# feldroop/genedex

Measured on AMD Instinct MI355X. Metric: queries/sec (count+locate), hg38-scale text, 100M len-50 reads, higher is better.
Workload: dtype u32

## Files before the change

### genedex_amd/csrc/search.hip

```cpp
#include <atomic>
#include <cstdlib>
#include <string>
#include <type_traits>

#include "common.hpp"
#include "kernels.hpp"

namespace gdx {

namespace {

constexpr int kBlock = 256;

struct QueryWindow {
    const uint64_t *words;
    uint64_t cur;
    uint64_t next;
    uint64_t cur_word;
    uint64_t first_word;

    __device__ __forceinline__ void init(const uint8_t *qbuf, uint64_t begin, uint64_t pos)
    {
        words = reinterpret_cast<const uint64_t *>(qbuf);
        first_word = begin >> 3;
// ... 2708 lines not shown
            s_pr[wave][at] = rem;
            s_pc[wave][at] = make_uint2(static_cast<uint32_t>(qcode), static_cast<uint32_t>(qcode >> 32));
        }
        n_parked += static_cast<uint32_t>(__popcll(mask));
    };
    auto goes_on = [&](const u32x4 &en, uint32_t tagd) __attribute__((always_inline)) {
        return (en.x & kSeedFound) == 0u && (en.x & kSeedOverflow) != 0u && (tagd >> kSeedDispShift) < kSeedMaxDisp;
    };
    auto parked_pass = [&]() __attribute__((always_inline)) {
        const uint32_t take = n_parked < 64u ? n_parked : 64u;
        const uint32_t first = n_parked - take;
        __builtin_amdgcn_wave_barrier();
        const bool mine = lane < take;
        uint32_t q = 0, bucket = 0, tagd = kNoTag, rem = 0;
        uint64_t qcode = 0;
        if (mine) {
            q = s_pq[wave][first + lane];
            bucket = s_pb[wave][first + lane];
            tagd = s_pt[wave][first + lane];
            rem = s_pr[wave][first + lane];
            const uint2 c = s_pc[wave][first + lane];
            qcode = (static_cast<uint64_t>(c.y) << 32) | c.x;
        }
        __builtin_amdgcn_wave_barrier();
        n_parked = first;
        s_bt[wave][lane] = make_uint2(bucket, tagd);
        const u32x4 en = gather();
        const bool again = mine && goes_on(en, tagd);
        const uint32_t kind = (mine && !again) ? finish(q, rem, qcode, en) : 0u;
        if (kind == 1u && tile_sums != nullptr) {
            const uint32_t t = q / kSumTile - tile0;
            if (t < 2u) atomicAdd(&s_tile_hits[t], 1u);
            else atomicAdd(&tile_sums[q / kSumTile], 1ull);
        }
        list_late(kind, q);
        park(again, q, bucket, tagd, rem, qcode);
    };

    const uint64_t n_ranges = (nq + range - 1) / range;
    for (uint64_t rg = blockIdx.x; rg < n_ranges; rg += gridDim.x) {
        const uint64_t base = rg * range;
        const uint32_t cnt = nq - base < range ? static_cast<uint32_t>(nq - base) : range;
        const uint32_t n_chunks = (cnt + 63u) >> 6;
        tile0 = static_cast<uint32_t>(base / kSumTile);
        uint64_t r_end = 0;
        uint32_t r_len = 0;
        bool r_on = false, r_load = false;
        uint32_t raw[kRaw];
#pragma unroll
        for (int i = 0; i < kRaw; i++) raw[i] = 0u;
        auto fetch = [&](uint32_t ch) __attribute__((always_inline)) {
            const uint32_t slot = ch * 64u + lane;
            r_on = ch < n_chunks && slot < cnt;
            r_load = false;
            if (!r_on) return;
            const uint64_t q = base + slot;
            uint64_t beg;
            if (kUniform) {
                beg = q * ulen;
                r_end = beg + ulen;
            } else {
                beg = qbeg[q];
                r_end = qend[q];
            }
            const uint64_t len = r_end - beg;
            r_len = len < (1ull << 21) ? static_cast<uint32_t>(len) : (1u << 21);
            r_load = r_len >= k && r_len < (1u << 21) && r_end >= kWin;
            if (!r_load) return;
            if (kXlate == 2) {
                const uint64_t bit = 2ull * (r_end - kWin);
                const uint32_t *p = qw + (bit >> 5);
                const u32x4_a4 v = *reinterpret_cast<const u32x4_a4 *>(p);
                raw[0] = v.x, raw[1] = v.y, raw[2] = v.z, raw[3] = v.w;
                raw[4] = p[4];
            } else {
                const uint32_t *p1 = qw + ((r_end - kWin) >> 2);
                const u32x4_a4 *p = reinterpret_cast<const u32x4_a4 *>(p1);
#pragma unroll
                for (int i = 0; i < 3; i++) {
                    const u32x4_a4 v = p[i];
                    raw[4 * i] = v.x, raw[4 * i + 1] = v.y, raw[4 * i + 2] = v.z, raw[4 * i + 3] = v.w;
                }
                raw[12] = p1[12];
                raw[13] = p1[13];
                raw[14] = ((r_end - kWin) & 3u) != 0u ? p1[14] : 0u;
            }
        };
        fetch(wave);
        for (uint32_t ch = wave; ch < n_chunks; ch += kWaves) {
            const uint32_t q = static_cast<uint32_t>(base + ch * 64u + lane);
            const bool on = r_on;
            bool left = on && !r_load;
            const uint32_t rem = r_len - k;
            uint32_t f0 = 0, f1 = 0, f2 = 0, f3 = 0;
            if (kXlate == 2) {
                const uint32_t sh = static_cast<uint32_t>(2ull * (r_end - kWin)) & 31u;
                f0 = __builtin_amdgcn_alignbit(raw[1], raw[0], sh);
                f1 = __builtin_amdgcn_alignbit(raw[2], raw[1], sh);
                f2 = __builtin_amdgcn_alignbit(raw[3], raw[2], sh);
                f3 = __builtin_amdgcn_alignbit(raw[4], raw[3], sh);
            } else {
                const uint32_t o = static_cast<uint32_t>(r_end - kWin) & 3u;
                const uint32_t lo = kWin - (r_len < span ? r_len : span);
                uint32_t bad = 0, c[14];
#pragma unroll
                for (uint32_t i = 0; i < 14; i++) {
                    const uint32_t bytes = __builtin_amdgcn_alignbyte(raw[i + 1], raw[i], o);
                    uint32_t b = 0;
                    c[i] = fast_pack4(sv, bytes, b);
                    const uint32_t m = 4u * i + 4u <= lo ? 0u : (4u * i >= lo ? 0xffffffffu : 0xffffffffu << (8u * (lo - 4u * i)));
                    bad |= b & m;
                }
                f0 = c[0] | (c[1] << 8) | (c[2] << 16) | (c[3] << 24);
                f1 = c[4] | (c[5] << 8) | (c[6] << 16) | (c[7] << 24);
                f2 = c[8] | (c[9] << 8) | (c[10] << 16) | (c[11] << 24);
                f3 = c[12] | (c[13] << 8);
                if (bad != 0u) left = on;
            }
            const uint64_t wq = (static_cast<uint64_t>(f1) << 32) | f0, wk = (static_cast<uint64_t>(f3) << 32) | f2;
            const uint64_t qcode0 = drop2 == 0u ? wq : (wq >> drop2) | (wk << (64u - drop2));
            const uint64_t key = (wk >> drop2) & ((1ull << (2u * k)) - 1ull);
            uint32_t tag = 0;
            const uint32_t bucket = seed_home(key, sv.tag_bits, sv.buckets, tag);
            const bool look = on && !left;
            s_bt[wave][lane] = look ? make_uint2(bucket, tag) : make_uint2(0u, kNoTag);
            s_qc[wave][lane] = make_uint2(static_cast<uint32_t>(qcode0), static_cast<uint32_t>(qcode0 >> 32));
            fetch(ch + kWaves);
            const u32x4 en = gather();
            uint32_t li = lane;
            asm volatile("" : "+v"(li));
            const uint2 qc2 = s_qc[wave][li];
            const uint64_t qcode = (static_cast<uint64_t>(qc2.y) << 32) | qc2.x;
            if (left) {
                if (state) state[q] = make_uint4(0u, 0u, 0u, 0u);
                if (out_compact) out_compact[q] = kCompactSee;
            }
            const bool again = look && goes_on(en, tag);
            const uint32_t kind = left ? kListLeft : ((look && !again) ? finish(q, rem, qcode, en) : 0u);
            list_slot(kind, ch * 64u + lane);
            if (tile_sums != nullptr) {
                const unsigned long long hm = __ballot(kind == 1u);
                if (lane == 0u && hm != 0ull)
                    atomicAdd(&s_tile_hits[static_cast<uint32_t>((base + ch * 64u) / kSumTile) - tile0], static_cast<uint32_t>(__popcll(hm)));
            }
            park(again, q, bucket, tag, rem, qcode);
            while (n_parked >= 64u) parked_pass();
        }
        if (rg + gridDim.x >= n_ranges)
            while (n_parked != 0u) parked_pass();
        flush_lists(base);
    }
}

template <int kXlate, bool kExact>
__global__ __launch_bounds__(kBlock) void seed_text_kernel4(
    SeedView sv, const uint8_t *__restrict__ qbuf, const uint64_t *__restrict__ qbeg, const uint32_t *__restrict__ list,
    const uint32_t *__restrict__ n_list, const uint2 *__restrict__ long_state, uint32_t long_stride,
    uint32_t *__restrict__ out_count, uint8_t *__restrict__ out_status, uint4 *__restrict__ out_rec,
    uint32_t *__restrict__ out_start, uint32_t *__restrict__ out_end, uint32_t *__restrict__ out_compact,
    uint4 *__restrict__ state, uint32_t *__restrict__ leftover, uint32_t *__restrict__ n_leftover, uint32_t ulen)
{
    constexpr uint32_t kGroup = 4, kGroups = kBlock / kGroup;
    __shared__ uint8_t s_dense[256];
    if (kXlate == 0) {
        for (int i = threadIdx.x; i < 256; i += kBlock) s_dense[i] = sv.io_to_dense[i];
        __syncthreads();
    }
    const uint32_t sub = threadIdx.x & (kGroup - 1u);
    const bool writer = sub == 0u;
    const uint64_t n = *n_list;
    for (uint64_t i = static_cast<uint64_t>(blockIdx.x) * kGroups + threadIdx.x / kGroup; i < n;
         i += static_cast<uint64_t>(gridDim.x) * kGroups) {
        const uint32_t q = list[i];
        uint32_t pos, rem;
        if (kExact) {
            pos = out_start[q];
            rem = out_end[q];
        } else {
            const uint2 st = long_state[static_cast<uint64_t>(q) * long_stride];
            pos = st.x;
            rem = st.y;
        }
        const uint64_t begin = query_begin(qbeg, ulen, q);
        const uint32_t rest = rem - 32u;
        uint32_t bad_q = 0, bad_t = 0;
        for (uint32_t done = 0; done < rest; done += 128u) {
            const uint32_t skip = done + 32u * sub;
            if (skip < rest) {
                const uint32_t e = rest - skip, n_c = e < 32u ? e : 32u, qs = e - n_c;
                const uint64_t at = begin + qs;
                const uint64_t s0 = static_cast<uint64_t>(pos) - rem + qs + 32u * kTextPadUnits;
                const uint32_t tb = static_cast<uint32_t>(s0 & 31u);
                const u32x4 *tu = sv.text_units + (s0 >> 5);
                uint64_t qc = 0;
                uint32_t inv = 0;
                u32x4 u0, u1;
                if (kXlate == 2) {
                    const uint16_t *up = reinterpret_cast<const uint16_t *>(qbuf) + (at >> 3);
                    const uint32_t sh = static_cast<uint32_t>(at & 7u) * 2u;
                    const uint32_t n_need = (static_cast<uint32_t>(at & 7u) + n_c + 7u) >> 3;
                    uint64_t lo64 = up[0];
                    uint32_t hi16 = 0;
                    if (n_need > 1u) lo64 |= static_cast<uint64_t>(up[1]) << 16;
                    if (n_need > 2u) lo64 |= static_cast<uint64_t>(up[2]) << 32;
                    if (n_need > 3u) lo64 |= static_cast<uint64_t>(up[3]) << 48;
                    if (n_need > 4u) hi16 = up[4];
                    u0 = tu[0];
                    u1 = tb != 0u ? tu[1] : u32x4{0u, 0u, 0u, 0u};
                    qc = sh != 0u ? (lo64 >> sh) | (static_cast<uint64_t>(hi16) << (64u - sh)) : lo64;
                } else {
                const uint64_t *wp = reinterpret_cast<const uint64_t *>(qbuf) + (at >> 3);
                const uint32_t sh = static_cast<uint32_t>(at & 7u) * 8u;
                const uint32_t n_need = (static_cast<uint32_t>(at & 7u) + n_c + 7u) >> 3;
                uint64_t w0 = wp[0], w1 = 0, w2 = 0, w3 = 0, w4 = 0;
                if (n_need > 1u) w1 = wp[1];
                if (n_need > 2u) w2 = wp[2];
                if (n_need > 3u) w3 = wp[3];
                if (n_need > 4u) w4 = wp[4];
                u0 = tu[0];
                u1 = tb != 0u ? tu[1] : u32x4{0u, 0u, 0u, 0u};
                if (sh != 0u) {
                    w0 = (w0 >> sh) | (w1 << (64u - sh));
                    w1 = (w1 >> sh) | (w2 << (64u - sh));
                    w2 = (w2 >> sh) | (w3 << (64u - sh));
                    w3 = (w3 >> sh) | (w4 << (64u - sh));
                }
                uint32_t b[8] = {0u, 0u, 0u, 0u, 0u, 0u, 0u, 0u};
                const uint32_t wd[8] = {static_cast<uint32_t>(w0), static_cast<uint32_t>(w0 >> 32), static_cast<uint32_t>(w1),
                                        static_cast<uint32_t>(w1 >> 32), static_cast<uint32_t>(w2), static_cast<uint32_t>(w2 >> 32),
                                        static_cast<uint32_t>(w3), static_cast<uint32_t>(w3 >> 32)};
#pragma unroll
                for (uint32_t g = 0; g < 8; g++) {
                    const uint32_t code = kXlate == 1 ? fast_pack4(sv, wd[g], b[g]) : fast_pack4_lds(s_dense, wd[g], b[g]);
                    qc |= static_cast<uint64_t>(code) << (8u * g);
                }
                const uint32_t full = n_c >> 2, part = n_c & 3u;
#pragma unroll
                for (uint32_t g = 0; g < 8; g++) {
                    const uint32_t bg = kXlate == 1 ? b[g] : (b[g] != 0u ? 0xffffffffu : 0u);
                    if (g < full) inv |= bg;
                    else if (g == full && part != 0u) inv |= bg & ((1u << (8u * part)) - 1u);
                }
                }
                const uint64_t c0 = static_cast<uint64_t>(u0.x) | (static_cast<uint64_t>(u0.y) << 32);
                const uint64_t c1 = static_cast<uint64_t>(u1.x) | (static_cast<uint64_t>(u1.y) << 32);
                const uint64_t tc = tb ? (c0 >> (2u * tb)) | (c1 << (64u - 2u * tb)) : c0;
                const uint32_t tm = tb ? (u0.z >> tb) | (u1.z << (32u - tb)) : u0.z;
                const uint64_t m64 = n_c == 32u ? ~0ull : (1ull << (2u * n_c)) - 1ull;
                const uint32_t m32 = n_c == 32u ? ~0u : (1u << n_c) - 1u;
                if (inv != 0u) bad_q = 1u;
                if (((qc ^ tc) & m64) != 0ull || (tm & m32) != 0u) bad_t = 1u;
            }
        }
        const bool left = group_max<kGroup>(bad_q) != 0u;
        const bool hit = group_max<kGroup>(bad_t) == 0u;
        if (kExact) {
            if (left || !hit) {
                if (writer) leftover[atomicAdd(n_leftover, 1u)] = q;
            } else {
                const uint32_t row = sv.isa[pos - rem];
                if (writer) {
                    out_start[q] = row;
                    out_end[q] = row + 1u;
                    if (out_count) out_count[q] = 1u;
                    if (out_status) out_status[q] = 0;
                }
            }
        } else if (writer) {
            if (left) {
                leftover[atomicAdd(n_leftover, 1u)] = q;
                if (state) state[q] = make_uint4(0u, 0u, 0u, 0u);
                if (out_compact) out_compact[q] = kCompactSee;
            } else {
                if (out_compact) out_compact[q] = hit ? pos - rem : kCompactNone;
                else if (out_rec) out_rec[q] = hit ? make_uint4(0u, 1u, pos - rem, kRecResolved) : make_uint4(0u, 0u, 0xffffffffu, 0u);
                if (out_count) out_count[q] = hit ? 1u : 0u;
                if (out_status) out_status[q] = 0;
            }
        }
    }
}

template <int kJump, int kMode>
__global__ __launch_bounds__(kBlock) __attribute__((amdgpu_waves_per_eu(7, 7))) void search_pair_packed_kernel4(GDX_SEARCH_ARGS)
{
    search_pair_body<0, 4, false, kJump, kMode, true>(GDX_SEARCH_FWD);
}
template <int kPolicy, int kJump, int kMode>
__global__ __launch_bounds__(kBlock) void search_pair_stats_kernel8(GDX_SEARCH_ARGS)
{
    search_pair_body<kPolicy, 8, true, kJump, kMode>(GDX_SEARCH_FWD);
}
template <int kPolicy, int kJump, int kMode>
__global__ __launch_bounds__(kBlock) void search_pair_stats_kernel4(GDX_SEARCH_ARGS)
{
    search_pair_body<kPolicy, 4, true, kJump, kMode>(GDX_SEARCH_FWD);
}

template <class Table, int kGroup, bool kPair>
__global__ __launch_bounds__(kBlock) void extend_front_kernel(IndexView ix, uint32_t *__restrict__ start,
                                                              uint32_t *__restrict__ end,
                                                              const uint8_t *__restrict__ io_symbols, uint64_t m,
                                                              uint8_t *__restrict__ out_status)
{
    const uint64_t stride = static_cast<uint64_t>(gridDim.x) * (kBlock / kGroup);
    const bool writer = (threadIdx.x % kGroup) == 0;
    for (uint64_t i = static_cast<uint64_t>(blockIdx.x) * (kBlock / kGroup) + threadIdx.x / kGroup; i < m; i += stride) {
        uint32_t lo = start[i], hi = end[i];
        const uint32_t c = ix.io_to_dense[io_symbols[i]];
        uint32_t status = GDX_Q_OK;
        if (c == 0) {
            status = GDX_Q_INVALID_SYMBOL;
        } else if (lo != hi) {
            if (kPair && c <= 4u) {
                PairTable::lf1<1, 8>(ix, c, lo, hi, lo, hi);
            } else {
                uint32_t rlo, rhi;
                Table::rank2(ix, c, lo, hi, rlo, rhi);
                const uint32_t cc = ix.count[c];
                lo = cc + rlo;
                hi = cc + rhi;
            }
            if (writer) {
                start[i] = lo;
                end[i] = hi;
            }
        }
        if (out_status && writer) out_status[i] = static_cast<uint8_t>(status);
    }
}

struct SegmentsOut {
    uint32_t *n_segments, *remaining, *length, *start, *end;
    uint8_t *status;
};

template <class Table, int kGroup, bool kPair, bool kText>
__global__ __launch_bounds__(kBlock) __attribute__((amdgpu_waves_per_eu((kText && kPair) ? 5 : ((kText || kGroup == 1) ? 6 : 7)))) void suffix_segments_kernel(
    IndexView ix, const uint8_t *__restrict__ qbuf, const uint64_t *__restrict__ qoff, uint64_t nq, uint32_t max_segments,
    SegmentsOut out)
{
    __shared__ uint8_t s_dense[256];
    __shared__ uint32_t s_count[257];
    for (int i = threadIdx.x; i < 256; i += kBlock) s_dense[i] = ix.io_to_dense[i];
    for (int i = threadIdx.x; i <= ix.sigma; i += kBlock) s_count[i] = ix.count[i];
    __syncthreads();

    const uint64_t stride = static_cast<uint64_t>(gridDim.x) * (kBlock / kGroup);
    const bool writer = (threadIdx.x % kGroup) == 0;
    const uint32_t sub = threadIdx.x % kGroup;
    const uint32_t depth = (ix.top != nullptr && ix.layout == 0) ? ix.top_depth : 0u;
    for (uint64_t q = static_cast<uint64_t>(blockIdx.x) * (kBlock / kGroup) + threadIdx.x / kGroup; q < nq; q += stride) {
        const uint64_t begin = qoff[q];
        const uint32_t m = static_cast<uint32_t>(qoff[q + 1] - begin);
        const uint64_t slot0 = q * max_segments;
        uint32_t e = m, n_seg = 0, status = GDX_Q_OK;
        while (e > 0u && n_seg < max_segments) {
            uint32_t lo = 0, hi = ix.n, len = 0;
            if (depth != 0u && e >= depth) {
                uint32_t a = 0, b = 0;
                for (uint32_t s = 0; s < depth; s++) {
                    const uint32_t c = s_dense[qbuf[begin + e - 1u - s]];
                    if (s < 8u) a |= c << (4u * (7u - s));
                    else b |= c << (4u * (15u - s));
                }
                uint32_t tlo, thi;
                if (top_lookup(ix, a, b, tlo, thi) && tlo != thi) {
                    lo = tlo;
                    hi = thi;
                    len = depth;
                }
            }
            QueryWindow win;
            win.init(qbuf, begin, begin + (e - len));
            bool text_open = kText;
            while (len < e) {
                if (kText && text_open && len != 0u && hi - lo == 1u) {
                    uint32_t p = ix.sa_full[lo];
                    bool blocked = false;
                    while (len < e) {
                        const uint32_t rem = e - len;
                        const uint64_t at = begin + rem;
                        const uint64_t t_hi = static_cast<uint64_t>(p) + 32u * kTextPadUnits - 1u - 8u * sub, t_lo = t_hi - 7u;
                        const u32x4 u_hi = ix.text_units[t_hi >> 5];
                        const u32x4 u_lo = (t_lo >> 5) != (t_hi >> 5) ? ix.text_units[t_lo >> 5] : u_hi;
                        uint32_t mine = 0, dirty = 0;
                        for (uint32_t k = 0; k < 8u; k++) {
                            const uint32_t j = 8u * sub + k;
                            if (j >= rem) break;
                            const uint32_t c = s_dense[qbuf[at - 1u - j]];
                            if (c - 1u >= 4u) {
                                dirty = 1u;
                                break;
                            }
                            const uint64_t t = t_hi - k;
                            const u32x4 u = (t >> 5) == (t_hi >> 5) ? u_hi : u_lo;
                            const uint32_t i = static_cast<uint32_t>(t & 31u);
                            const uint32_t code = ((i < 16u ? u.x >> (2u * i) : u.y >> (2u * (i - 16u)))) & 3u;
                            if (((u.z >> i) & 1u) != 0u || code != c - 1u) break;
                            mine++;
                        }
                        const uint32_t v = mine | (dirty << 8);
                        uint32_t total = 0, stop = 0, stop_dirty = 0;
#pragma unroll
                        for (int l = 0; l < kGroup; l++) {
                            const uint32_t vl = kGroup == 1 ? v : static_cast<uint32_t>(__shfl(static_cast<int>(v), l, kGroup));
                            if (stop == 0u) {
                                total += vl & 0xffu;
                                if ((vl & 0xffu) < 8u) {
                                    stop = 1u;
                                    stop_dirty = vl >> 8;
                                }
                            }
                        }
                        p -= total;
                        len += total;
                        if (stop != 0u) {
                            blocked = stop_dirty == 0u;
                            break;
                        }
                    }
                    lo = ix.isa[p];
                    hi = lo + 1u;
                    if (blocked || len == e) break;
                    text_open = false;
                    win.init(qbuf, begin, begin + (e - len));
                    continue;
                }
                const uint32_t c = s_dense[win.get(begin + (e - len) - 1u)];
                if (c == 0u) {
                    status = GDX_Q_INVALID_SYMBOL;
                    break;
                }
// ... 357 lines not shown
void ZeroSet::flush(hipStream_t stream)
{
    if (n == 0) return;
    ZeroSegments z{};
    uint64_t total = 0;
    for (int i = 0; i < n; i++) {
        z.p[i] = p[i];
        total += words[i];
        if (total > 0xffffffffull) fail(GDX_ERR_INVALID_ARGUMENT, "internal: ZeroSet regions beyond 16 GB");
        z.end[i] = static_cast<uint32_t>(total);
    }
    z.n = n;
    const uint64_t blocks = (total + kBlock * 4 - 1) / (kBlock * 4);
    hipLaunchKernelGGL(zero_segments_kernel, dim3(static_cast<unsigned>(blocks < 1024 ? blocks : 1024)), dim3(kBlock), 0, stream, z);
    n = 0;
}

__global__ __launch_bounds__(kBlock) void fill_uniform_offsets_kernel(uint64_t *__restrict__ off, uint64_t n, uint32_t ulen)
{
    const uint64_t stride = static_cast<uint64_t>(gridDim.x) * kBlock;
    for (uint64_t i = static_cast<uint64_t>(blockIdx.x) * kBlock + threadIdx.x; i < n; i += stride) off[i] = i * ulen;
}

__global__ __launch_bounds__(kBlock) void fill_uniform_offsets_list_kernel(uint64_t *__restrict__ off, const uint32_t *__restrict__ list,
                                                                          const uint32_t *__restrict__ n_list, uint32_t ulen)
{
    const uint64_t n = *n_list;
    for (uint64_t i = static_cast<uint64_t>(blockIdx.x) * kBlock + threadIdx.x; i < n; i += static_cast<uint64_t>(gridDim.x) * kBlock) {
        const uint64_t q = list[i];
        off[q] = q * ulen;
        off[q + 1] = (q + 1) * ulen;
    }
}

__global__ __launch_bounds__(kBlock) void tile_sums_lists_kernel(const uint4 *__restrict__ rec, const uint32_t *__restrict__ compact,
                                                                 uint32_t max_hits, const uint32_t *__restrict__ left,
                                                                 const uint32_t *__restrict__ n_left, const uint32_t *__restrict__ lng,
                                                                 const uint32_t *__restrict__ n_lng,
                                                                 unsigned long long *__restrict__ tile_sums,
                                                                 unsigned long long *__restrict__ rest)
{
    const uint64_t stride = static_cast<uint64_t>(gridDim.x) * kBlock;
    const uint64_t nl = *n_left, ng = *n_lng;
    const uint64_t n = nl + ng, n_round = (n + 63) / 64 * 64;
    unsigned long long open_slots = 0;
    for (uint64_t i = static_cast<uint64_t>(blockIdx.x) * kBlock + threadIdx.x; i < n_round; i += stride) {
        unsigned long long c = 0;
        uint32_t tile = 0xffffffffu;
        if (i < n) {
            const bool is_left = i < nl;
            const uint32_t q = is_left ? left[i] : lng[i - nl];
            const uint32_t c4 = compact[q];
            tile = q / kSumTile;
            if (c4 == kCompactSee) {
                if (is_left) {
                    const uint2 v = *reinterpret_cast<const uint2 *>(rec + q);
                    const uint32_t m = v.y - v.x;
                    c = (max_hits != 0u && m > max_hits) ? 0ull : static_cast<unsigned long long>(m);
                    open_slots += c;
                }
            } else {
                c = c4 == kCompactNone ? 0ull : 1ull;
            }
        }
        const uint32_t tile0 = static_cast<uint32_t>(__builtin_amdgcn_readfirstlane(static_cast<int>(tile)));
        if (__ballot(tile != tile0 && c != 0ull) == 0ull) {
            unsigned long long sum = tile == tile0 ? c : 0ull;
            for (int off = 32; off > 0; off >>= 1) sum += __shfl_xor(sum, off);
            if ((threadIdx.x & 63u) == 0u && sum != 0ull && tile0 != 0xffffffffu) atomicAdd(&tile_sums[tile0], sum);
        } else if (c != 0ull) {
            atomicAdd(&tile_sums[tile], c);
        }
    }
    for (int off = 32; off > 0; off >>= 1) open_slots += __shfl_xor(open_slots, off);
    if ((threadIdx.x & 63u) == 0u && open_slots != 0ull) atomicAdd(rest, open_slots);
}

template <int V, int... Rest, class F>
static void with_int(int v, F &&f)
{
    if constexpr (sizeof...(Rest) != 0) {
        if (v != V) return with_int<Rest...>(v, f);
    }
    f(std::integral_constant<int, V>());
}
template <class F> static void with_bool(bool b, F &&f) { b ? f(std::true_type()) : f(std::false_type()); }
template <class F> static void with_jump_bytes(int jump_bytes, F &&f) { with_int<32, 16, 8>(jump_bytes, f); }
template <class F> static void with_xlate(int xlate, F &&f) { with_int<2, 1, 0>(xlate, f); }

static int env_int(const char *name, int absent) { const char *e = getenv(name); return e ? atoi(e) : absent; }
static long env_long(const char *name, long absent) { const char *e = getenv(name); return e ? atol(e) : absent; }
static bool env_set(const char *name) { return getenv(name) != nullptr; }

struct SearchKnobs {
    long grid = env_long("GDX_SEARCH_GRID", 0);
    unsigned pad = static_cast<unsigned>(env_long("GDX_SEARCH_PAD", 0));
    int lanes = env_int("GDX_SEARCH_LANES", 4) == 8 ? 8 : 4;
    int policy = env_int("GDX_LOAD_POLICY", 0);
    int schedule = [] { const char *e = getenv("GDX_SEARCH_SCHEDULE"); return (e && e[0] == '0') ? 0 : 1; }();
    int defer = env_int("GDX_SEARCH_DEFER", 0);
    int fast = env_int("GDX_SEARCH_FAST", -1);
    int exact = env_int("GDX_SEARCH_EXACT", -1);
    int seed = env_int("GDX_SEARCH_SEED", -1);
    int text = env_int("GDX_SEARCH_TEXT", 1);
    bool no_perm = env_set("GDX_SEARCH_NO_PERM");
    bool fast_stats = env_set("GDX_SEARCH_FAST_STATS");
    int seed_lean = env_int("GDX_SEARCH_SEED_LEAN", 1);
    int seed_chain = env_int("GDX_SEARCH_SEED_CHAIN", 1);
    int seed_packed = env_int("GDX_SEARCH_SEED_PACKED", 1);
    int seed_lane = env_int("GDX_SEED_LANE", 1);
    int seed_cursor = env_int("GDX_SEARCH_SEED_CURSOR", 1);
    unsigned seed_pad = static_cast<unsigned>(env_long("GDX_SEED_PAD", 0));
    uint32_t seed_lane_range = static_cast<uint32_t>(env_long("GDX_SEED_LANE_RANGE", 0));
    unsigned seed_list_blocks = static_cast<unsigned>(env_long("GDX_SEED_LIST_BLOCKS", 1792));
};
static const SearchKnobs &search_knobs() { static const SearchKnobs knobs; return knobs; }

struct SearchSettings {
    int variant;
    int lanes;
    int policy;
    int schedule;
    uint32_t defer_after;
    int fast;
    bool exact;
    bool seed;
    bool perm;
    int xlate;
    bool text_route;

    SearchSettings(const IndexView &ix, const QueryOptions &qo, const SearchKnobs &k, const SearchCall &c)
    {
        variant = qo.search_variant >= 0 ? qo.search_variant : search_variant();
        lanes = (qo.search_lanes == 4 || qo.search_lanes == 8) ? qo.search_lanes : k.lanes;
        policy = (qo.load_policy >= 0 ? qo.load_policy : k.policy) == 1 ? 1 : 0;
        schedule = qo.length_schedule >= 0 ? (qo.length_schedule != 0) : k.schedule;
        defer_after = c.d_step_stats != nullptr ? 0u : static_cast<uint32_t>(qo.search_defer_after >= 0 ? qo.search_defer_after : k.defer);
        const int f = k.fast >= 0 ? k.fast : qo.search_fast;
        fast = f == 0 ? 0 : (f == 2 ? 2 : 1);
        exact = k.exact >= 0 ? k.exact != 0 : qo.search_exact != 0;
        seed = k.seed >= 0 ? k.seed != 0 : qo.search_seed != 0;
        perm = ix.perm_ok && !k.no_perm;
        xlate = c.packed ? 2 : (perm ? 1 : 0);
        text_route = ix.jump == nullptr && ix.sa_full != nullptr && ix.isa != nullptr && ix.text_units != nullptr && k.text != 0;
    }
};

struct ListGrid { unsigned blocks; uint32_t range; };
static unsigned range_blocks(uint64_t nq, uint32_t range, uint64_t cap)
{
    const uint64_t ranges = (nq + range - 1) / range;
    return static_cast<unsigned>(ranges < cap ? ranges : cap);
}
static ListGrid range_grid(uint64_t nq, uint32_t range_cap, long grid_override)
{
    uint64_t per_block = (nq + 1791) / 1792;
    per_block = (per_block + 63) / 64 * 64;
    const uint32_t range = static_cast<uint32_t>(per_block > range_cap ? range_cap : per_block);
    return {grid_override > 0 ? static_cast<unsigned>(grid_override) : range_blocks(nq, range, 1u << 20), range};
}
static ListGrid short_list_grid(uint64_t nq, unsigned cap = 8192) { return {range_blocks(nq, 256, cap), 256}; }
static unsigned group_grid(uint64_t nq, uint64_t groups_per_block, long grid_override)
{
    const uint64_t needed = (nq + groups_per_block - 1) / groups_per_block;
    uint64_t blocks = (nq + groups_per_block * 48 - 1) / (groups_per_block * 48);
    if (blocks < 1792) blocks = 1792;
    if (blocks > 65536) blocks = 65536;
    if (blocks > needed) blocks = needed;
    if (grid_override > 0) blocks = static_cast<uint64_t>(grid_override);
    return static_cast<unsigned>(blocks);
}

static SeedView seed_view(const IndexView &ix, const uint32_t *isa)
{
    return SeedView{ix.seed, ix.text_units, isa, ix.io_to_dense, ix.seed_buckets, ix.seed_k, ix.seed_tag_bits,
                    ix.perm_code_lo, ix.perm_code_hi, ix.perm_exp_lo, ix.perm_exp_hi, ix.perm_mask};
}
static VerifyView verify_view(const IndexView &ix)
{
    const bool entry_sa = ix.jump != nullptr && ix.jump_bytes == 32;
    const uint32_t max_rows = (ix.sa_full != nullptr || entry_sa) ? 4u : 1u;
    return VerifyView{ix.top, ix.text_units, ix.sa_full, entry_sa ? ix.jump : nullptr, ix.lines, ix.sb_offsets, ix.count,
                      ix.sa_samples, ix.border_keys, ix.border_vals, ix.io_to_dense, ix.top_depth, ix.n, ix.n_texts,
                      ix.sa_inv, ix.sa_rot, ix.sa_limit, max_rows, ix.perm_code_lo, ix.perm_code_hi, ix.perm_exp_lo,
                      ix.perm_exp_hi, ix.perm_mask, ix.seed, ix.seed_buckets, ix.seed_k, ix.seed_tag_bits, ix.seed_pairs, ix.seed_quads};
}
static ExactView exact_view(const IndexView &ix, bool with_seed)
{
    return ExactView{ix.top, ix.jump, ix.pair_lines, ix.io_to_dense, ix.top_depth, ix.n, static_cast<uint32_t>(ix.depth),
                     ix.perm_code_lo, ix.perm_code_hi, ix.perm_exp_lo, ix.perm_exp_hi, ix.perm_mask, ix.sa_full, ix.isa,
                     ix.text_units, with_seed ? ix.seed : nullptr, ix.seed_buckets, ix.seed_k, ix.seed_tag_bits};
}
static FastView fast_view(const IndexView &ix)
{
    return FastView{ix.top, ix.jump, ix.io_to_dense, ix.top_depth, ix.sa_inv, ix.sa_rot, ix.sa_limit,
                    ix.perm_code_lo, ix.perm_code_hi, ix.perm_exp_lo, ix.perm_exp_hi, ix.perm_mask};
}

struct SeedLaunch {
    SeedView sv;
    ListGrid grid;
    unsigned lds = 0;
    uint4 *rec = nullptr;
    uint32_t *start = nullptr, *end = nullptr;
    uint32_t *first = nullptr, *lng = nullptr;
    uint4 *state = nullptr;
    uint32_t *compact = nullptr;
    uint2 *long_state = nullptr;
    uint32_t long_stride = 0, state_packed = 0;
};

struct SearchChain {
    ZeroSet zs;
    CursorArgs ca;
    bool leftover_list = false;
    uint32_t *seed_list = nullptr;
    uint32_t seed_state_packed = 0;
    bool compact_by_seed = false;
    uint32_t *fold_left = nullptr, *fold_long = nullptr;
    uint64_t *d_uniform_off = nullptr;
    bool sparse_offsets = false;
    ListGrid all{}, exact{}, general{};
    CursorArgs ca_exact, ca_general;
};

struct SearchLauncher {
    const IndexView &ix;
    SearchCall c;
    hipStream_t stream;
    const SearchKnobs &k;
    const SearchSettings s;
    const uint64_t nq;
    const bool seed_pairs;
    const long lane_blocks_cap;
    uint32_t ulen = 0;
    SearchChain st;

    uint32_t *counted_list(int slot, ZeroSet *zs)
    {
        uint32_t *list = static_cast<uint32_t *>(stream_scratch(stream, slot, (nq + 4) * sizeof(uint32_t)));
        if (zs != nullptr) zs->add(list, sizeof(uint32_t));
        else GDX_HIP(hipMemsetAsync(list, 0, sizeof(uint32_t), stream));
        return list;
    }
    void print_left(const char *path, const uint32_t *n_list, const char *next)
    {
        uint32_t n_left = 0;
        GDX_HIP(hipMemcpyAsync(&n_left, n_list, sizeof(uint32_t), hipMemcpyDeviceToHost, stream));
        GDX_HIP(hipStreamSynchronize(stream));
        fprintf(stderr, "gdx: %s path left %u of %llu queries to the %s kernel\n", path, n_left, static_cast<unsigned long long>(nq), next);
    }
    template <int kXlate, bool kExact>
    void launch_seed_text(const SeedLaunch &a)
    {
        hipLaunchKernelGGL((seed_text_kernel4<kXlate, kExact>), dim3(range_blocks(nq, kBlock / 4, 8192)), dim3(kBlock), 0, stream, a.sv,
                           c.d_qbuf, c.d_qbeg, a.lng + 4, a.lng, a.long_state, a.long_stride, c.d_count, c.d_status, a.rec, a.start,
                           a.end, a.compact, a.state, a.first + 4, a.first, ulen);
    }
    template <int kXlate, bool kExact>
    void launch_seed_and_text(const SeedLaunch &a)
    {
        hipLaunchKernelGGL((search_seed_kernel4<kXlate, kExact>), dim3(a.grid.blocks), dim3(kBlock), a.lds, stream, a.sv, c.d_qbuf,
                           c.d_qbeg, c.d_qend, nq, c.d_count, c.d_status, a.rec, a.start, a.end, a.grid.range, a.first + 4, a.first,
                           a.state, a.compact, a.lng + 4, a.lng, a.long_state, a.long_stride, a.state_packed, ulen, CursorArgs());
        launch_seed_text<kXlate, kExact>(a);
    }
    template <bool kSeed>
    void launch_verify(ListGrid grid, uint32_t *left, uint32_t *list, const uint4 *state, uint32_t wide)
    {
        const VerifyView vv = verify_view(ix);
        with_xlate(s.xlate, [&](auto X) {
            hipLaunchKernelGGL((search_verify_kernel4<decltype(X)::value, kSeed>), dim3(grid.blocks), dim3(kBlock), 0, stream, vv,
                               c.d_qbuf, c.d_qbeg, c.d_qend, nq, c.d_count, c.d_status, c.d_rec, grid.range, left + 4, left,
                               list ? list + 4 : nullptr, list, ulen, state, wide, state != nullptr ? st.seed_state_packed : 0u);
        });
    }

    void seed_front(ListGrid v_grid, uint32_t *d_left)
    {
        const bool pair_general = s.variant == 2 && ix.pair_lines != nullptr;
        const bool to_fast = k.seed_lean != 0 && k.seed_chain != 0 && pair_general && ix.top != nullptr && ix.top_depth >= 1u &&
                             ix.jump != nullptr && ix.top_depth >= static_cast<uint32_t>(ix.depth) && s.lanes == 4 && s.policy == 0 &&
                             s.fast != 0;
        const bool to_verify_packed = !to_fast && pair_general && k.seed_lean != 0;
        st.seed_state_packed = (to_fast || to_verify_packed) && c.d_rec != nullptr && k.seed_packed != 0 ? 1u : 0u;
        if (st.seed_state_packed != 0u && !to_fast && (ix.seed_pairs != nullptr || ix.seed_quads != nullptr) && seed_pairs)
            st.seed_state_packed = 2u;
        if (k.seed_lean == 0) {
            st.zs.flush(stream);
            return launch_verify<true>(v_grid, d_left, nullptr, nullptr, 0u);
        }
        SeedLaunch a{seed_view(ix, nullptr), v_grid, k.seed_pad, c.d_rec};
        a.first = counted_list(12, &st.zs);
        const bool to_verify_with_state = !to_fast && pair_general && c.d_rec != nullptr;
        a.state = (to_fast || to_verify_with_state) ? c.d_rec : nullptr;
        a.compact = c.d_compact;
        a.lng = counted_list(13, &st.zs);
        a.long_state = c.d_rec != nullptr ? reinterpret_cast<uint2 *>(c.d_rec) : static_cast<uint2 *>(stream_scratch(stream, 14, nq * sizeof(uint2)));
        a.long_stride = c.d_rec != nullptr ? 2u : 1u;
        a.state_packed = st.seed_state_packed;
        const bool lane_kernel = k.seed_lane != 0 && s.xlate != 0 && ix.seed_k <= 24u && ix.seed_k >= 8u &&
                                 (reinterpret_cast<uintptr_t>(c.d_qbuf) & 3u) == 0;
        unsigned long long *fold = nullptr;
        if (lane_kernel && c.d_tile_sums != nullptr && c.d_tile_rest != nullptr && c.d_compact != nullptr) {
            fold = c.d_tile_sums;
            st.zs.add(fold, ((nq + kSumTile - 1) / kSumTile) * sizeof(unsigned long long));
            st.fold_left = a.first;
            st.fold_long = a.lng;
        }
        const uint32_t lane_range = k.seed_lane_range >= 64u && k.seed_lane_range <= kLaneRange ? k.seed_lane_range / 64u * 64u
                                    : (v_grid.range < kLaneRange ? v_grid.range : kLaneRange);
        if (lane_range % 64u != 0u) fail(GDX_ERR_INVALID_ARGUMENT, "internal: the lane kernel's ranges are multiples of 64");
        unsigned lane_blocks = range_blocks(nq, lane_range, 1u << 20);
        if (lane_blocks_cap > 0 && static_cast<unsigned long>(lane_blocks_cap) < lane_blocks) lane_blocks = static_cast<unsigned>(lane_blocks_cap);
        st.zs.flush(stream);
        if (lane_kernel) {
            with_int<2, 1>(s.xlate, [&](auto X) {
                constexpr int kX = decltype(X)::value;
                with_bool(ulen != 0u, [&](auto U) {
                    hipLaunchKernelGGL((search_seed_lane_kernel<kX, decltype(U)::value>), dim3(lane_blocks), dim3(kBlock), a.lds, stream,
                                       a.sv, c.d_qbuf, c.d_qbeg, c.d_qend, nq, c.d_count, c.d_status, c.d_rec, lane_range, a.first + 4,
                                       a.first, a.state, a.compact, a.lng + 4, a.lng, a.long_state, a.long_stride, a.state_packed, ulen, fold);
                });
                launch_seed_text<kX, false>(a);
            });
        } else {
            with_xlate(s.xlate, [&](auto X) { launch_seed_and_text<decltype(X)::value, false>(a); });
        }
        st.compact_by_seed = true;
        if (to_fast) {
            st.seed_list = a.first;
            return;
        }
        if (to_verify_with_state) st.ca.resume_state = a.state;
        launch_verify<true>(short_list_grid(nq, k.seed_list_blocks), d_left, a.first, to_verify_with_state ? a.state : nullptr,
                            to_verify_with_state ? 1u : 0u);
    }

    void front()
    {
        const bool clean_call = c.mode == 1 && ix.layout == 0 && ix.text_units != nullptr && ix.n_searchable >= 4 &&
                                c.d_step_stats == nullptr && c.d_hint == nullptr && c.d_start == nullptr &&
                                c.d_end == nullptr && st.ca.active_in == nullptr && nq < 0xffffffffull;
        const bool seed = clean_call && ix.seed != nullptr && ix.seed_k >= static_cast<uint32_t>(ix.depth) && s.seed;
        const bool verify = !seed && clean_call && ix.top != nullptr && ix.top_depth >= 1u && ix.jump == nullptr &&
                            ix.top_depth >= static_cast<uint32_t>(ix.depth) && s.fast != 0;
        if (!seed && !verify) return;
        const ListGrid v_grid = range_grid(nq, kMaxRange, 0);
        uint32_t *d_left = counted_list(11, &st.zs);
        if (seed) {
            seed_front(v_grid, d_left);
        } else {
            st.zs.flush(stream);
            launch_verify<false>(v_grid, d_left, nullptr, nullptr, 0u);
        }
        uint32_t *next = st.seed_list ? st.seed_list : d_left;
        if (k.fast_stats) print_left(seed ? "seed" : "verify", next, "next");
        st.ca.active_in = next + 4;
        st.ca.n_active_in = next;
        st.leftover_list = true;
    }

    void uniform_offsets(bool sparse)
    {
        st.d_uniform_off = static_cast<uint64_t *>(stream_scratch(stream, 15, (nq + 1) * sizeof(uint64_t)));
        if (!sparse)
            hipLaunchKernelGGL(fill_uniform_offsets_kernel, dim3(grid_for_items(nq + 1)), dim3(kBlock), 0, stream, st.d_uniform_off,
                               nq + 1, c.uniform_len);
        c.d_qbeg = st.d_uniform_off;
        c.d_qend = st.d_uniform_off + 1;
        c.uniform_len = 0;
        st.sparse_offsets = sparse;
    }
    void offsets_for_list(const uint32_t *list, const uint32_t *n_list)
    {
        if (st.sparse_offsets && list != nullptr)
            hipLaunchKernelGGL(fill_uniform_offsets_list_kernel, dim3(1024), dim3(kBlock), 0, stream, st.d_uniform_off, list, n_list, ulen);
    }

    void pair_seed_exact()
    {
        SeedLaunch a{seed_view(ix, ix.isa), st.all};
        a.first = counted_list(12, nullptr);
        a.start = c.d_start;
        a.end = c.d_end;
        a.lng = counted_list(13, nullptr);
        with_xlate(s.xlate, [&](auto X) { launch_seed_and_text<decltype(X)::value, true>(a); });
        st.ca_exact.active_in = a.first + 4;
        st.ca_exact.n_active_in = a.first;
        st.exact = short_list_grid(nq);
    }
    void pair_seed_cursor()
    {
        uint32_t *d_first = counted_list(12, nullptr);
        SeedView sv = seed_view(ix, ix.isa);
        sv.n = ix.n;
        with_int<1, 0>(s.perm ? 1 : 0, [&](auto X) {
            hipLaunchKernelGGL((search_seed_kernel4<decltype(X)::value, true, true>), dim3(st.all.blocks), dim3(kBlock), 0, stream, sv,
                               c.d_qbuf, c.d_qbeg, c.d_qend, nq, c.d_count, c.d_status, nullptr, c.d_start, c.d_end, st.all.range,
                               d_first + 4, d_first, nullptr, nullptr, nullptr, nullptr, nullptr, 0u, 0u, 0u, st.ca);
        });
        st.ca_exact.active_in = d_first + 4;
        st.ca_exact.n_active_in = d_first;
        st.exact = short_list_grid(nq);
    }
    void pair_exact(bool seed_in_kernel)
    {
        uint32_t *d_left = counted_list(11, nullptr);
// ... 323 lines not shown
```

Measured before the change: 26.46 billion.

## Rebalance seed text verification with per-wave LDS work rings of query pieces

Replaces the fixed four-lanes-per-query text verification with a per-wave scheme: each wave loads 64 list entries, splits every query's remaining suffix into 32-character pieces, and queues them in an LDS ring that is drained 64 pieces at a time. Mismatch flags are combined through LDS atomics, and the next chunk's state is prefetched into a double buffer. Leftover appends are aggregated per wave with a ballot, and the grid is sized to resident occupancy with a waves-per-EU hint. The goal is to remove idle lanes caused by variable suffix lengths, at the cost of more LDS traffic, wave barriers and extra bookkeeping.

```diff
diff --git a/genedex_amd/csrc/search.hip b/genedex_amd/csrc/search.hip
--- a/genedex_amd/csrc/search.hip
+++ b/genedex_amd/csrc/search.hip
@@ -2884,27 +2884,48 @@
     }
 }
 
+constexpr uint32_t kTextPer = 4;
+constexpr uint32_t kTextRing = 64 + 64 * kTextPer;
+template <int kXlate>
+constexpr int kTextWavesPerEu = kXlate == 2 ? 8 : 6;
 template <int kXlate, bool kExact>
-__global__ __launch_bounds__(kBlock) void seed_text_kernel4(
+__global__ __launch_bounds__(kBlock) __attribute__((amdgpu_waves_per_eu(kTextWavesPerEu<kXlate>))) void seed_text_kernel4(
     SeedView sv, const uint8_t *__restrict__ qbuf, const uint64_t *__restrict__ qbeg, const uint32_t *__restrict__ list,
     const uint32_t *__restrict__ n_list, const uint2 *__restrict__ long_state, uint32_t long_stride,
     uint32_t *__restrict__ out_count, uint8_t *__restrict__ out_status, uint4 *__restrict__ out_rec,
     uint32_t *__restrict__ out_start, uint32_t *__restrict__ out_end, uint32_t *__restrict__ out_compact,
     uint4 *__restrict__ state, uint32_t *__restrict__ leftover, uint32_t *__restrict__ n_leftover, uint32_t ulen)
 {
-    constexpr uint32_t kGroup = 4, kGroups = kBlock / kGroup;
+    constexpr uint32_t kWaves = kBlock / 64, kPer = kTextPer, kRing = kTextRing;
+    constexpr uint32_t kPieceBits = 17, kOwnerShift = kPieceBits, kSlotShift = kPieceBits + 6, kFirstPiece = 1u << (kSlotShift + 1);
+    const uint64_t n = *n_list;
+    if (n == 0ull) return;
     __shared__ uint8_t s_dense[256];
+    __shared__ uint32_t s_ring[kWaves][kRing];
+    __shared__ uint4 s_rd[2][kWaves][64];
+    __shared__ uint32_t s_q[2][kWaves][64], s_flag[2][kWaves][64];
     if (kXlate == 0) {
         for (int i = threadIdx.x; i < 256; i += kBlock) s_dense[i] = sv.io_to_dense[i];
         __syncthreads();
     }
-    const uint32_t sub = threadIdx.x & (kGroup - 1u);
-    const bool writer = sub == 0u;
-    const uint64_t n = *n_list;
-    for (uint64_t i = static_cast<uint64_t>(blockIdx.x) * kGroups + threadIdx.x / kGroup; i < n;
-         i += static_cast<uint64_t>(gridDim.x) * kGroups) {
-        const uint32_t q = list[i];
-        uint32_t pos, rem;
+    const uint32_t lane = threadIdx.x & 63u, wave = __builtin_amdgcn_readfirstlane(threadIdx.x >> 6);
+    const uint64_t n_chunks = (n + 63u) >> 6;
+    const uint64_t stride = static_cast<uint64_t>(gridDim.x) * kWaves;
+    const unsigned long long lanes_below = (1ull << lane) - 1ull;
+    uint32_t head = 0, n_queued = 0;
+
+    auto wave_sync = [&]() __attribute__((always_inline)) {
+        __builtin_amdgcn_fence(__ATOMIC_RELEASE, "wavefront");
+        __builtin_amdgcn_wave_barrier();
+        __builtin_amdgcn_fence(__ATOMIC_ACQUIRE, "wavefront");
+    };
+    auto load_entry = [&](uint64_t ch) __attribute__((always_inline)) -> uint32_t {
+        const uint64_t i = ch * 64u + lane;
+        return i < n ? list[i] : 0u;
+    };
+    auto load_state = [&](uint64_t ch, uint32_t q, uint32_t &pos, uint32_t &rem, uint64_t &begin) __attribute__((always_inline)) {
+        pos = 0u, rem = 0u, begin = 0ull;
+        if (ch * 64u + lane >= n) return;
         if (kExact) {
             pos = out_start[q];
             rem = out_end[q];
@@ -2913,104 +2934,179 @@
             pos = st.x;
             rem = st.y;
         }
-        const uint64_t begin = query_begin(qbeg, ulen, q);
-        const uint32_t rest = rem - 32u;
-        uint32_t bad_q = 0, bad_t = 0;
-        for (uint32_t done = 0; done < rest; done += 128u) {
-            const uint32_t skip = done + 32u * sub;
-            if (skip < rest) {
-                const uint32_t e = rest - skip, n_c = e < 32u ? e : 32u, qs = e - n_c;
-                const uint64_t at = begin + qs;
-                const uint64_t s0 = static_cast<uint64_t>(pos) - rem + qs + 32u * kTextPadUnits;
-                const uint32_t tb = static_cast<uint32_t>(s0 & 31u);
-                const u32x4 *tu = sv.text_units + (s0 >> 5);
-                uint64_t qc = 0;
-                uint32_t inv = 0;
-                u32x4 u0, u1;
-                if (kXlate == 2) {
-                    const uint16_t *up = reinterpret_cast<const uint16_t *>(qbuf) + (at >> 3);
-                    const uint32_t sh = static_cast<uint32_t>(at & 7u) * 2u;
-                    const uint32_t n_need = (static_cast<uint32_t>(at & 7u) + n_c + 7u) >> 3;
-                    uint64_t lo64 = up[0];
-                    uint32_t hi16 = 0;
-                    if (n_need > 1u) lo64 |= static_cast<uint64_t>(up[1]) << 16;
-                    if (n_need > 2u) lo64 |= static_cast<uint64_t>(up[2]) << 32;
-                    if (n_need > 3u) lo64 |= static_cast<uint64_t>(up[3]) << 48;
-                    if (n_need > 4u) hi16 = up[4];
-                    u0 = tu[0];
-                    u1 = tb != 0u ? tu[1] : u32x4{0u, 0u, 0u, 0u};
-                    qc = sh != 0u ? (lo64 >> sh) | (static_cast<uint64_t>(hi16) << (64u - sh)) : lo64;
-                } else {
-                const uint64_t *wp = reinterpret_cast<const uint64_t *>(qbuf) + (at >> 3);
-                const uint32_t sh = static_cast<uint32_t>(at & 7u) * 8u;
-                const uint32_t n_need = (static_cast<uint32_t>(at & 7u) + n_c + 7u) >> 3;
-                uint64_t w0 = wp[0], w1 = 0, w2 = 0, w3 = 0, w4 = 0;
-                if (n_need > 1u) w1 = wp[1];
-                if (n_need > 2u) w2 = wp[2];
-                if (n_need > 3u) w3 = wp[3];
-                if (n_need > 4u) w4 = wp[4];
+        begin = query_begin(qbeg, ulen, q);
+    };
+    auto pass = [&](uint32_t take) __attribute__((always_inline)) {
+        wave_sync();
+        uint32_t at = head + lane;
+        if (at >= kRing) at -= kRing;
+        const uint32_t en = lane < take ? s_ring[wave][at] : 0u;
+        if (n_queued > 64u) {
+            const uint32_t behind = head + 64u >= kRing ? head + 64u - kRing : head + 64u;
+            if ((__builtin_amdgcn_readfirstlane(s_ring[wave][behind]) & kFirstPiece) == 0u)
+                take = 63u - static_cast<uint32_t>(__builtin_clzll(__ballot((en & kFirstPiece) != 0u)));
+        }
+        if (lane < take) {
+            const uint32_t piece = en & ((1u << kPieceBits) - 1u), owner = (en >> kOwnerShift) & 63u, slot = (en >> kSlotShift) & 1u;
+            const uint4 rd = s_rd[slot][wave][owner];
+            const uint64_t begin = (static_cast<uint64_t>(rd.y) << 32) | rd.x;
+            const uint32_t pos = rd.z, rem = rd.w, rest = rem - 32u;
+            const uint32_t e = rest - 32u * piece, n_c = e < 32u ? e : 32u, qs = e - n_c;
+            const uint64_t at_q = begin + qs;
+            const uint64_t s0 = static_cast<uint64_t>(pos) - rem + qs + 32u * kTextPadUnits;
+            const uint32_t tb = static_cast<uint32_t>(s0 & 31u);
+            const u32x4 *tu = sv.text_units + (s0 >> 5);
+            uint64_t qc = 0;
+            uint32_t inv = 0;
+            u32x4 u0, u1;
+            if (kXlate == 2) {
+                const uint16_t *up = reinterpret_cast<const uint16_t *>(qbuf) + (at_q >> 3);
+                const uint32_t sh = static_cast<uint32_t>(at_q & 7u) * 2u;
+                const uint32_t n_need = (static_cast<uint32_t>(at_q & 7u) + n_c + 7u) >> 3;
                 u0 = tu[0];
                 u1 = tb != 0u ? tu[1] : u32x4{0u, 0u, 0u, 0u};
-                if (sh != 0u) {
-                    w0 = (w0 >> sh) | (w1 << (64u - sh));
-                    w1 = (w1 >> sh) | (w2 << (64u - sh));
-                    w2 = (w2 >> sh) | (w3 << (64u - sh));
-                    w3 = (w3 >> sh) | (w4 << (64u - sh));
-                }
-                uint32_t b[8] = {0u, 0u, 0u, 0u, 0u, 0u, 0u, 0u};
-                const uint32_t wd[8] = {static_cast<uint32_t>(w0), static_cast<uint32_t>(w0 >> 32), static_cast<uint32_t>(w1),
-                                        static_cast<uint32_t>(w1 >> 32), static_cast<uint32_t>(w2), static_cast<uint32_t>(w2 >> 32),
-                                        static_cast<uint32_t>(w3), static_cast<uint32_t>(w3 >> 32)};
+                uint64_t lo64 = up[0];
+                uint32_t hi16 = 0;
+                if (n_need > 1u) lo64 |= static_cast<uint64_t>(up[1]) << 16;
+                if (n_need > 2u) lo64 |= static_cast<uint64_t>(up[2]) << 32;
+                if (n_need > 3u) lo64 |= static_cast<uint64_t>(up[3]) << 48;
+                if (n_need > 4u) hi16 = up[4];
+                qc = sh != 0u ? (lo64 >> sh) | (static_cast<uint64_t>(hi16) << (64u - sh)) : lo64;
+            } else {
+            const uint64_t *wp = reinterpret_cast<const uint64_t *>(qbuf) + (at_q >> 3);
+            const uint32_t sh = static_cast<uint32_t>(at_q & 7u) * 8u;
+            const uint32_t n_need = (static_cast<uint32_t>(at_q & 7u) + n_c + 7u) >> 3;
+            u0 = tu[0];
+            u1 = tb != 0u ? tu[1] : u32x4{0u, 0u, 0u, 0u};
+            uint64_t w0 = wp[0], w1 = 0, w2 = 0, w3 = 0, w4 = 0;
+            if (n_need > 1u) w1 = wp[1];
+            if (n_need > 2u) w2 = wp[2];
+            if (n_need > 3u) w3 = wp[3];
+            if (n_need > 4u) w4 = wp[4];
+            if (sh != 0u) {
+                w0 = (w0 >> sh) | (w1 << (64u - sh));
+                w1 = (w1 >> sh) | (w2 << (64u - sh));
+                w2 = (w2 >> sh) | (w3 << (64u - sh));
+                w3 = (w3 >> sh) | (w4 << (64u - sh));
+            }
+            uint32_t b[8] = {0u, 0u, 0u, 0u, 0u, 0u, 0u, 0u};
+            const uint32_t wd[8] = {static_cast<uint32_t>(w0), static_cast<uint32_t>(w0 >> 32), static_cast<uint32_t>(w1),
+                                    static_cast<uint32_t>(w1 >> 32), static_cast<uint32_t>(w2), static_cast<uint32_t>(w2 >> 32),
+                                    static_cast<uint32_t>(w3), static_cast<uint32_t>(w3 >> 32)};
 #pragma unroll
-                for (uint32_t g = 0; g < 8; g++) {
-                    const uint32_t code = kXlate == 1 ? fast_pack4(sv, wd[g], b[g]) : fast_pack4_lds(s_dense, wd[g], b[g]);
-                    qc |= static_cast<uint64_t>(code) << (8u * g);
-                }
-                const uint32_t full = n_c >> 2, part = n_c & 3u;
+            for (uint32_t g = 0; g < 8; g++) {
+                const uint32_t code = kXlate == 1 ? fast_pack4(sv, wd[g], b[g]) : fast_pack4_lds(s_dense, wd[g], b[g]);
+                qc |= static_cast<uint64_t>(code) << (8u * g);
+            }
+            const uint32_t full = n_c >> 2, part = n_c & 3u;
 #pragma unroll
-                for (uint32_t g = 0; g < 8; g++) {
-                    const uint32_t bg = kXlate == 1 ? b[g] : (b[g] != 0u ? 0xffffffffu : 0u);
-                    if (g < full) inv |= bg;
-                    else if (g == full && part != 0u) inv |= bg & ((1u << (8u * part)) - 1u);
-                }
-                }
-                const uint64_t c0 = static_cast<uint64_t>(u0.x) | (static_cast<uint64_t>(u0.y) << 32);
-                const uint64_t c1 = static_cast<uint64_t>(u1.x) | (static_cast<uint64_t>(u1.y) << 32);
-                const uint64_t tc = tb ? (c0 >> (2u * tb)) | (c1 << (64u - 2u * tb)) : c0;
-                const uint32_t tm = tb ? (u0.z >> tb) | (u1.z << (32u - tb)) : u0.z;
-                const uint64_t m64 = n_c == 32u ? ~0ull : (1ull << (2u * n_c)) - 1ull;
-                const uint32_t m32 = n_c == 32u ? ~0u : (1u << n_c) - 1u;
-                if (inv != 0u) bad_q = 1u;
-                if (((qc ^ tc) & m64) != 0ull || (tm & m32) != 0u) bad_t = 1u;
-            }
-        }
-        const bool left = group_max<kGroup>(bad_q) != 0u;
-        const bool hit = group_max<kGroup>(bad_t) == 0u;
+            for (uint32_t g = 0; g < 8; g++) {
+                const uint32_t bg = kXlate == 1 ? b[g] : (b[g] != 0u ? 0xffffffffu : 0u);
+                if (g < full) inv |= bg;
+                else if (g == full && part != 0u) inv |= bg & ((1u << (8u * part)) - 1u);
+            }
+            }
+            const uint64_t c0 = static_cast<uint64_t>(u0.x) | (static_cast<uint64_t>(u0.y) << 32);
+            const uint64_t c1 = static_cast<uint64_t>(u1.x) | (static_cast<uint64_t>(u1.y) << 32);
+            const uint64_t tc = tb ? (c0 >> (2u * tb)) | (c1 << (64u - 2u * tb)) : c0;
+            const uint32_t tm = tb ? (u0.z >> tb) | (u1.z << (32u - tb)) : u0.z;
+            const uint64_t m64 = n_c == 32u ? ~0ull : (1ull << (2u * n_c)) - 1ull;
+            const uint32_t m32 = n_c == 32u ? ~0u : (1u << n_c) - 1u;
+            const uint32_t fl = (inv != 0u ? 1u : 0u) | ((((qc ^ tc) & m64) != 0ull || (tm & m32) != 0u) ? 2u : 0u);
+            if (fl != 0u) atomicOr(&s_flag[slot][wave][owner], fl);
+        }
+        head += take;
+        if (head >= kRing) head -= kRing;
+        n_queued -= take;
+    };
+    auto append_left = [&](bool mine, uint32_t q) __attribute__((always_inline)) {
+        const unsigned long long mask = __ballot(mine);
+        if (mask == 0ull) return;
+        const int leader = __ffsll(static_cast<long long>(mask)) - 1;
+        uint32_t first = 0;
+        if (static_cast<int>(lane) == leader) first = atomicAdd(n_leftover, static_cast<uint32_t>(__popcll(mask)));
+        first = __shfl(first, leader);
+        if (mine) leftover[first + static_cast<uint32_t>(__popcll(mask & lanes_below))] = q;
+    };
+    auto finish = [&](uint32_t slot) __attribute__((always_inline)) {
+        wave_sync();
+        const uint4 rd = s_rd[slot][wave][lane];
+        const uint32_t q = s_q[slot][wave][lane], fl = s_flag[slot][wave][lane];
+        const uint32_t pos = rd.z, rem = rd.w;
+        const bool on = rem != 0u;
+        const bool left = (fl & 1u) != 0u;
+        const bool hit = (fl & 2u) == 0u;
         if (kExact) {
-            if (left || !hit) {
-                if (writer) leftover[atomicAdd(n_leftover, 1u)] = q;
-            } else {
-                const uint32_t row = sv.isa[pos - rem];
-                if (writer) {
-                    out_start[q] = row;
-                    out_end[q] = row + 1u;
-                    if (out_count) out_count[q] = 1u;
-                    if (out_status) out_status[q] = 0;
-                }
-            }
-        } else if (writer) {
-            if (left) {
-                leftover[atomicAdd(n_leftover, 1u)] = q;
+            const bool found = on && !left && hit;
+            uint32_t row = 0;
+            if (found) row = sv.isa[pos - rem];
+            append_left(on && !found, q);
+            if (found) {
+                out_start[q] = row;
+                out_end[q] = row + 1u;
+                if (out_count) out_count[q] = 1u;
+                if (out_status) out_status[q] = 0;
+            }
+        } else {
+            append_left(on && left, q);
+            if (on && left) {
                 if (state) state[q] = make_uint4(0u, 0u, 0u, 0u);
                 if (out_compact) out_compact[q] = kCompactSee;
-            } else {
+            } else if (on) {
                 if (out_compact) out_compact[q] = hit ? pos - rem : kCompactNone;
                 else if (out_rec) out_rec[q] = hit ? make_uint4(0u, 1u, pos - rem, kRecResolved) : make_uint4(0u, 0u, 0xffffffffu, 0u);
                 if (out_count) out_count[q] = hit ? 1u : 0u;
                 if (out_status) out_status[q] = 0;
             }
         }
-    }
+    };
+
+    uint64_t ch = static_cast<uint64_t>(blockIdx.x) * kWaves + wave;
+    if (ch >= n_chunks) return;
+    uint32_t q1 = load_entry(ch), q2 = load_entry(ch + stride);
+    uint32_t pos1, rem1;
+    uint64_t beg1;
+    load_state(ch, q1, pos1, rem1, beg1);
+    uint32_t slot = 0;
+    bool have_prev = false;
+    for (; ch < n_chunks; ch += stride) {
+        s_rd[slot][wave][lane] = make_uint4(static_cast<uint32_t>(beg1), static_cast<uint32_t>(beg1 >> 32), pos1, rem1);
+        s_q[slot][wave][lane] = q1;
+        s_flag[slot][wave][lane] = 0u;
+        const uint32_t n_pieces = rem1 > 32u ? (rem1 - 32u + 31u) >> 5 : 0u;
+        q1 = q2;
+        load_state(ch + stride, q1, pos1, rem1, beg1);
+        q2 = load_entry(ch + 2u * stride);
+        const uint32_t prev_left = n_queued;
+        bool ran = false;
+        for (uint32_t done = 0;; done += kPer) {
+            const uint32_t cnt = n_pieces > done ? (n_pieces - done < kPer ? n_pieces - done : kPer) : 0u;
+            const unsigned long long b0 = __ballot((cnt & 1u) != 0u), b1 = __ballot((cnt & 2u) != 0u), b2 = __ballot((cnt & 4u) != 0u);
+            if ((b0 | b1 | b2) == 0ull) break;
+            const uint32_t before = static_cast<uint32_t>(__popcll(b0 & lanes_below)) + 2u * static_cast<uint32_t>(__popcll(b1 & lanes_below)) +
+                                    4u * static_cast<uint32_t>(__popcll(b2 & lanes_below));
+            uint32_t at = head + n_queued + before;
+            if (at >= kRing) at -= kRing;
+#pragma unroll
+            for (uint32_t j = 0; j < kPer; j++) {
+                if (j < cnt) s_ring[wave][at] = (done + j) | (lane << kOwnerShift) | (slot << kSlotShift) | (j == 0u ? kFirstPiece : 0u);
+                if (++at == kRing) at = 0u;
+            }
+            n_queued += static_cast<uint32_t>(__popcll(b0)) + 2u * static_cast<uint32_t>(__popcll(b1)) + 4u * static_cast<uint32_t>(__popcll(b2));
+            while (n_queued >= 64u) {
+                pass(64u);
+                ran = true;
+            }
+        }
+        if (have_prev) {
+            if (!ran && prev_left != 0u) pass(n_queued);
+            finish(slot ^ 1u);
+        }
+        have_prev = true;
+        slot ^= 1u;
+    }
+    if (n_queued != 0u) pass(n_queued);
+    finish(slot ^ 1u);
 }
 
 template <int kJump, int kMode>
@@ -3674,6 +3770,16 @@
     const uint64_t ranges = (nq + range - 1) / range;
     return static_cast<unsigned>(ranges < cap ? ranges : cap);
 }
+template <class Kernel>
+static unsigned resident_blocks(Kernel kernel)
+{
+    int per_cu = 0, dev = 0;
+    hipDeviceProp_t prop;
+    if (hipOccupancyMaxActiveBlocksPerMultiprocessor(&per_cu, kernel, kBlock, 0) != hipSuccess || per_cu < 1) per_cu = 4;
+    if (hipGetDevice(&dev) != hipSuccess || hipGetDeviceProperties(&prop, dev) != hipSuccess || prop.multiProcessorCount < 1)
+        return static_cast<unsigned>(per_cu) * 256u;
+    return static_cast<unsigned>(per_cu) * static_cast<unsigned>(prop.multiProcessorCount);
+}
 static ListGrid range_grid(uint64_t nq, uint32_t range_cap, long grid_override)
 {
     uint64_t per_block = (nq + 1791) / 1792;
@@ -3775,7 +3881,8 @@
     template <int kXlate, bool kExact>
     void launch_seed_text(const SeedLaunch &a)
     {
-        hipLaunchKernelGGL((seed_text_kernel4<kXlate, kExact>), dim3(range_blocks(nq, kBlock / 4, 8192)), dim3(kBlock), 0, stream, a.sv,
+        static const unsigned resident = resident_blocks(seed_text_kernel4<kXlate, kExact>);
+        hipLaunchKernelGGL((seed_text_kernel4<kXlate, kExact>), dim3(range_blocks(nq, kBlock, resident)), dim3(kBlock), 0, stream, a.sv,
                            c.d_qbuf, c.d_qbeg, a.lng + 4, a.lng, a.long_state, a.long_stride, c.d_count, c.d_status, a.rec, a.start,
                            a.end, a.compact, a.state, a.first + 4, a.first, ulen);
     }
```

After: 26.21 billion, median of 2. About the same (-0.9%).
